# akanazawa/human_dynamics

Hardware: NVIDIA H100
Metric: frames/sec (ResNet->f_movie->SMPL LBS) (higher is better)
Workload: dtype f32 (wgmma 3x fp16 head/remainder split, fp32 two-level accumulate)

## Files before the change

### human_dynamics_b200/csrc/conv_tc.cu

```cuda
#include <cuda.h>
#include <cuda_fp16.h>
#include <cstdlib>
#include "conv_common.cuh"
#include "tc_ptx.cuh"

namespace hd {
namespace {

constexpr int BM = 128;
constexpr int A_TILE_BYTES = BM * 128;
constexpr int BOX_BYTES = 64 * 128;
constexpr int W_PROD = 8;
constexpr int STAGE_OUT = 1, STAGE_PAIR = 2;

using namespace ptx;

template <bool SPLIT, bool HALF, bool ASPLIT, int BN, bool RES = false, bool SHORT = false>
struct Cfg {
  static_assert(BN == 64 || (BN == 128 && HALF && ASPLIT), "128-wide N tiles: pre-split fp16 path only");
  static_assert(!RES || ASPLIT, "residual by TMA: pre-split fp16 path only");
  static_assert(!SHORT || (BN == 64 && HALF && ASPLIT), "two CTAs per SM: 64-wide pre-split fp16 tiles only");
  static constexpr int CTAS = SHORT ? 2 : 1;
  static constexpr int PROD_THREADS = BN == 128 || SHORT ? 128 : 256;
  static constexpr int NUM_THREADS = 256 + PROD_THREADS;
  static constexpr int ROW_STEP = PROD_THREADS / 8;
  static constexpr int ROWS = BM / ROW_STEP;
  static constexpr int PROD_REGS = SHORT ? 32 : BN == 128 ? 40 : 104, CONS_REGS = SHORT ? 104 : BN == 128 ? 232 : 152;
  static_assert(CTAS * (256 * CONS_REGS + PROD_THREADS * PROD_REGS) <= 65536, "setmaxnreg split beyond the register file");
  static constexpr int NACC = BN / 2;
  static constexpr int STAGES = SHORT ? 1 : BN == 128 ? (RES ? 2 : 3) : (RES ? 3 : 4);
  static constexpr int BKE = HALF ? 64 : 32;
  static constexpr int B_TILE_BYTES = BN * 128;
  static constexpr int B_OFFSET = (SPLIT ? 2 : 1) * A_TILE_BYTES;
  static constexpr int STAGE_BYTES = (SPLIT ? 2 : 1) * (A_TILE_BYTES + B_TILE_BYTES);
  static constexpr int RES_OFFSET = STAGES * STAGE_BYTES;
  static constexpr int RES_SLOT_BYTES = RES || SHORT ? 64 * BN * 4 : 0;
  static constexpr int STG_OFFSET = SHORT ? RES_OFFSET : RES_OFFSET + 2 * RES_SLOT_BYTES;
  static constexpr int STG_BYTES = ASPLIT ? 2 * BOX_BYTES : 0;
  static_assert(!SHORT || STG_BYTES == RES_SLOT_BYTES, "SHORT: the staging buffer is the residual slot");
  static constexpr int BAR_OFFSET = SHORT ? RES_OFFSET + 2 * RES_SLOT_BYTES : STG_OFFSET + 2 * STG_BYTES;
  static constexpr int SMEM_BYTES = BAR_OFFSET + 128 + 1024;
  static_assert(SMEM_BYTES <= 232448, "dynamic shared memory beyond the 227 KB a CTA can opt into");
  static_assert(CTAS * (SMEM_BYTES + 1024) <= 233472, "CTAS CTAs (and the 1 KB each reserves) beyond an SM's 228 KB");
  static constexpr int PF = HALF ? 2 : 3;
  static constexpr int V = HALF ? 2 : 1;
};

template <int R>
struct RowState {
  int n[R], iy[R], ix[R];
};

template <bool SPLIT, int PCH, bool HALF, bool GATHER, bool ASPLIT, int BN, bool RES, bool SHORT>
__global__ void __launch_bounds__((Cfg<SPLIT, HALF, ASPLIT, BN, RES, SHORT>::NUM_THREADS), (Cfg<SPLIT, HALF, ASPLIT, BN, RES, SHORT>::CTAS))
conv_gemm_tc_kernel(const ConvParams p, const __grid_constant__ CUtensorMap tmap_hi, const __grid_constant__ CUtensorMap tmap_lo,
                    const __grid_constant__ CUtensorMap tmap_res, const __grid_constant__ CUtensorMap tmap_out,
                    const __grid_constant__ CUtensorMap tmap_out_hi, const __grid_constant__ CUtensorMap tmap_out_lo, const int stage) {
  using C = Cfg<SPLIT, HALF, ASPLIT, BN, RES, SHORT>;
  constexpr bool MEM_STAMPS = BN == 128 || SHORT;
  constexpr int BKE = C::BKE, PF = C::PF, V = C::V, STAGES = C::STAGES, R = C::ROWS, RS = C::ROW_STEP, NA = C::NACC;
  extern __shared__ uint8_t smem_raw[];
  const uint32_t smem_base = (smem_u32(smem_raw) + 1023u) & ~1023u;
  uint8_t *smem = smem_raw + (smem_base - smem_u32(smem_raw));
  const uint32_t bar_base = smem_base + C::BAR_OFFSET;
  auto full_bar = [&](int s) { return bar_base + 8u * s; };
  auto empty_bar = [&](int s) { return bar_base + 8u * (STAGES + s); };
  auto res_bar = [&](int g) { return bar_base + 8u * (2 * STAGES + g); };

  const int warp = threadIdx.x >> 5, lane = threadIdx.x & 31;
  const int num_k = (GATHER ? p.K_pad : p.K) / BKE;
  const int tiles_n = (p.Cout + BN - 1) / BN;
  const int num_tiles = ((p.M + BM - 1) / BM) * tiles_n;
  const int my_tiles = (num_tiles - (int)blockIdx.x + (int)gridDim.x - 1) / (int)gridDim.x;

  if (threadIdx.x == 0) {
    for (int s = 0; s < STAGES; ++s) {
      mbar_init(full_bar(s), ASPLIT ? C::PROD_THREADS + 1 : 9);
      mbar_init(empty_bar(s), 8);
    }
    if (RES) for (int g = 0; g < 2; ++g) mbar_init(res_bar(g), 1);
    asm volatile("fence.mbarrier_init.release.cluster;" ::: "memory");
  }
  __syncthreads();
  const int xmode = p.dbg ? (int)p.dbg[15] : 0;

  if (warp >= W_PROD) {
    asm volatile("setmaxnreg.dec.sync.aligned.u32 %0;" ::"n"(C::PROD_REGS));
    const int t = threadIdx.x - W_PROD * 32;
    const int j = t & 7;
    const int rb = t >> 3;
    const uint32_t sw_off = (uint32_t)((j ^ (rb & 7)) << 4);
    const bool prof = p.dbg != nullptr && blockIdx.x == 0 && t == 0;
    long long t_wait = 0, t_start = prof && !MEM_STAMPS ? clock64() : 0;
    if (MEM_STAMPS && prof) { p.dbg[0] = clock64(); p.dbg[1] = 0; }
    auto wait_empty = [&](int s, uint32_t ph) {
      if (MEM_STAMPS && prof) p.dbg[1] -= clock64();
      const long long tw0 = !MEM_STAMPS && prof ? clock64() : 0;
      mbar_wait(empty_bar(s), ph ^ 1u);
      if (!MEM_STAMPS && prof) t_wait += clock64() - tw0;
      if (MEM_STAMPS && prof) p.dbg[1] += clock64();
    };
    const int total = my_tiles * num_k;
    auto load_b = [&](int s, int ti, int kc) {
      if (t != 0) return;
      const int n0 = (((int)blockIdx.x + ti * (int)gridDim.x) % tiles_n) * BN;
      const uint32_t b_hi = smem_base + s * C::STAGE_BYTES + C::B_OFFSET;
      if (xmode & 2) { mbar_arrive(full_bar(s)); return; }
      const int boxes = (BN == 128 && n0 + 64 < p.Cout) ? 2 : 1;
      mbar_arrive_expect_tx(full_bar(s), (SPLIT ? 2 : 1) * boxes * BOX_BYTES);
      for (int b = 0; b < boxes; ++b) {
        tma_load_2d(b_hi + b * BOX_BYTES, &tmap_hi, full_bar(s), kc * BKE, n0 + 64 * b);
        if (SPLIT) tma_load_2d(b_hi + C::B_TILE_BYTES + b * BOX_BYTES, &tmap_lo, full_bar(s), kc * BKE, n0 + 64 * b);
      }
    };

    auto enter_tile = [&](int ti, RowState<R> &rs) {
      const int tile = (int)blockIdx.x + ti * (int)gridDim.x;
      const int m0 = (tile / tiles_n) * BM;
      const int hw = p.Ho * p.Wo;
#pragma unroll
      for (int i = 0; i < R; ++i) {
        const int m = m0 + rb + RS * i;
        if (m < p.M) {
          const int n = m / hw;
          const int r = m - n * hw;
          const int oy = r / p.Wo, ox = r - oy * p.Wo;
          rs.n[i] = n; rs.iy[i] = oy * p.stride - p.pad_t; rs.ix[i] = ox * p.stride - p.pad_l;
        } else {
          rs.n[i] = -1; rs.iy[i] = 0; rs.ix[i] = 0;
        }
      }
    };
    if constexpr (ASPLIT) {
      const __half *ihi = reinterpret_cast<const __half *>(p.in_hi);
      const __half *ilo = reinterpret_cast<const __half *>(p.in_lo);
      if (SHORT || (!p.planes && p.KH * p.KW <= 32 && (long long)p.n_img * p.H * p.W * p.in_ld < (1ll << 31))) {
        const uint32_t off0 = (uint32_t)rb * 128u + sw_off;
        int base[R];
        uint32_t mask[R];
        int kc = 0, ti = 0, tap = 0, ci0 = 0, kx = 0, ky = 0, tap_off = 0;
        for (int q = 0; q < total; ++q) {
          if (kc == 0) {
            const int tile = (int)blockIdx.x + ti * (int)gridDim.x;
            const int m0 = (tile / tiles_n) * BM + rb;
            const int hw = p.Ho * p.Wo;
#pragma unroll
            for (int i = 0; i < R; ++i) {
              const int m = m0 + RS * i;
              uint32_t mk = 0;
              int b = 0;
              if (m < p.M) {
                const int n = m / hw;
                const int r = m - n * hw;
                const int oy = r / p.Wo, ox = r - oy * p.Wo;
                const int iy0 = oy * p.stride - p.pad_t, ix0 = ox * p.stride - p.pad_l;
                b = ((n * p.H + iy0) * p.W + ix0) * p.in_ld + j * 8;
                int t = 0;
                for (int yy = 0; yy < p.KH; ++yy)
                  for (int xx = 0; xx < p.KW; ++xx, ++t)
                    if ((unsigned)(iy0 + yy) < (unsigned)p.H && (unsigned)(ix0 + xx) < (unsigned)p.W) mk |= 1u << t;
              }
              base[i] = SHORT && !(mk & 1u) ? -1 : b;
              mask[i] = mk;
            }
            tap = 0; ci0 = 0; kx = 0; ky = 0; tap_off = 0;
          }
          const int s = q % STAGES;
          const uint32_t ph = (uint32_t)(q / STAGES) & 1u;
          wait_empty(s, ph);
          load_b(s, ti, kc);
          const uint32_t a_hi = smem_base + s * C::STAGE_BYTES + off0;
          const int eo = SHORT ? ci0 : tap_off + ci0;
#pragma unroll
          for (int i = 0; i < R; ++i) {
            const bool ok = SHORT ? base[i] >= 0 : (mask[i] >> tap) & 1u;
            const int e = ok ? base[i] + eo : 0;
            cp_async16(a_hi + i * RS * 128, ihi + e, ok ? 16u : 0u);
            if (SPLIT) cp_async16(a_hi + A_TILE_BYTES + i * RS * 128, ilo + e, ok ? 16u : 0u);
          }
          asm volatile("cp.async.mbarrier.arrive.noinc.shared::cta.b64 [%0];" ::"r"(full_bar(s)) : "memory");
          ci0 += BKE;
          if (ci0 == p.Cin) {
            ci0 = 0; ++tap;
            if (++kx == p.KW) { kx = 0; ++ky; }
            tap_off = (ky * p.W + kx) * p.in_ld;
          }
          if (++kc == num_k) { kc = 0; ++ti; }
        }
      } else if (!SHORT && p.planes && (long long)p.n_img * p.H * p.W * p.in_ld < (1ll << 31)) {
        const uint32_t off0 = (uint32_t)rb * 128u + sw_off;
        const int jt = j >> 2;
        const int row_step = 2 * p.W * (int)p.in_ld;
        int base[R];
        int kc = 0, ti = 0;
        for (int q = 0; q < total; ++q) {
          if (kc == 0) {
            const int tile = (int)blockIdx.x + ti * (int)gridDim.x;
            const int m0 = (tile / tiles_n) * BM + rb;
            const int hw = p.Ho * p.Wo;
#pragma unroll
            for (int i = 0; i < R; ++i) {
              const int m = m0 + RS * i;
              int b = -1;
              if (m < p.M) {
                const int n = m / hw;
                const int r = m - n * hw;
                const int oy = r / p.Wo, ox = r - oy * p.Wo;
                b = ((n * p.H + oy * p.stride + jt) * p.W + ox * p.stride) * (int)p.in_ld + (j & 3) * 8;
              }
              base[i] = b;
            }
          }
          const int s = q % STAGES;
          const uint32_t ph = (uint32_t)(q / STAGES) & 1u;
          wait_empty(s, ph);
          load_b(s, ti, kc);
          const uint32_t a_hi = smem_base + s * C::STAGE_BYTES + off0;
          const bool tap_ok = 2 * kc + jt < 7;
          const int eo = kc * row_step;
#pragma unroll
          for (int i = 0; i < R; ++i) {
            const bool ok = tap_ok && base[i] >= 0;
            const int e = ok ? base[i] + eo : 0;
            cp_async16_ca(a_hi + i * RS * 128, ihi + e, ok ? 16u : 0u);
            if (SPLIT) cp_async16_ca(a_hi + A_TILE_BYTES + i * RS * 128, ilo + e, ok ? 16u : 0u);
          }
          asm volatile("cp.async.mbarrier.arrive.noinc.shared::cta.b64 [%0];" ::"r"(full_bar(s)) : "memory");
          if (++kc == num_k) { kc = 0; ++ti; }
        }
      } else if (!SHORT) {
      RowState<R> rs;
      int kc = 0, ti = 0;
      for (int q = 0; q < total; ++q) {
        if (kc == 0) enter_tile(ti, rs);
        const int s = q % STAGES;
        const uint32_t ph = (uint32_t)(q / STAGES) & 1u;
        wait_empty(s, ph);
        load_b(s, ti, kc);
        const int kb = kc * BKE;
        const int tap = p.planes ? 2 * kc + (j >> 2) : kb / p.Cin;
        const int ci = p.planes ? (j & 3) * 8 : kb - tap * p.Cin + j * 8;
        const int ky = tap / p.KW, kx = tap - ky * p.KW;
        const bool tap_ok = !p.planes || tap < 7;
        const uint32_t a_hi = smem_base + s * C::STAGE_BYTES, a_lo = a_hi + A_TILE_BYTES;
#pragma unroll
        for (int i = 0; i < R; ++i) {
          const int iy = rs.iy[i] + ky, ix = rs.ix[i] + kx;
          const bool ok = tap_ok && rs.n[i] >= 0 && iy >= 0 && iy < p.H && ix >= 0 && ix < p.W;
          const size_t e = ok ? ((size_t)((size_t)rs.n[i] * p.H + iy) * p.W + ix) * p.in_ld + ci : 0;
          const uint32_t off = (uint32_t)(rb + RS * i) * 128u + sw_off;
          if (p.planes) {
            cp_async16_ca(a_hi + off, ihi + e, ok ? 16u : 0u);
            if (SPLIT) cp_async16_ca(a_lo + off, ilo + e, ok ? 16u : 0u);
          } else {
            cp_async16(a_hi + off, ihi + e, ok ? 16u : 0u);
            if (SPLIT) cp_async16(a_lo + off, ilo + e, ok ? 16u : 0u);
          }
        }
        asm volatile("cp.async.mbarrier.arrive.noinc.shared::cta.b64 [%0];" ::"r"(full_bar(s)) : "memory");
        if (++kc == num_k) { kc = 0; ++ti; }
      }
      }
      cp_async_commit();
      cp_async_wait<0>();
      if (prof) { p.dbg[0] = clock64() - (MEM_STAMPS ? p.dbg[0] : t_start); if (!MEM_STAMPS) p.dbg[1] = t_wait; }
    } else {
    RowState<R> pf_rs, st_rs;
    float4 ring[PF][4 * V];
    uint32_t vmask[PF];
    int pf_kc = 0, pf_ti = 0;
    auto prefetch = [&](float4 *dst, uint32_t &vm) {
      if (pf_kc == 0) enter_tile(pf_ti, pf_rs);
      if (GATHER) {
        const int seg = p.KW * p.Cin, segp = (seg + 7) & ~7;
        const int g8 = (pf_kc * BKE + j * (4 * V)) / 8;
        const int gpr = segp >> 3;
        const int ky = g8 / gpr, r0 = (g8 - ky * gpr) * 8;
        vm = 0;
#pragma unroll
        for (int i = 0; i < 4; ++i) {
          const int iy = pf_rs.iy[i] + ky;
          const bool okr = pf_rs.n[i] >= 0 && ky < p.KH && iy >= 0 && iy < p.H;
          const int c0 = pf_rs.ix[i] * p.Cin + r0;
          const float *src = p.in + ((size_t)((size_t)(okr ? pf_rs.n[i] : 0) * p.H + (okr ? iy : 0)) * p.W) * p.in_ld + c0;
          const int rowlen = p.W * p.Cin;
          float xs[8];
#pragma unroll
          for (int e = 0; e < 8; ++e) {
            const bool ok = okr && (r0 + e) < seg && (c0 + e) >= 0 && (c0 + e) < rowlen;
            xs[e] = ok ? __ldg(src + e) : 0.f;
          }
          dst[i * V] = make_float4(xs[0], xs[1], xs[2], xs[3]);
          dst[i * V + V - 1] = make_float4(xs[4], xs[5], xs[6], xs[7]);
          if (pf_rs.n[i] >= 0) vm |= 1u << i;
        }
        if (++pf_kc == num_k) { pf_kc = 0; ++pf_ti; }
        return;
      }
      const int kb = pf_kc * BKE;
      const int tap = kb / p.Cin, ci = kb - tap * p.Cin + j * (4 * V);
      const int ky = tap / p.KW, kx = tap - ky * p.KW;
      vm = 0;
#pragma unroll
      for (int i = 0; i < 4; ++i) {
        const int iy = pf_rs.iy[i] + ky, ix = pf_rs.ix[i] + kx;
        const bool ok = pf_rs.n[i] >= 0 && iy >= 0 && iy < p.H && ix >= 0 && ix < p.W;
        if (ok && !(xmode & 4)) {
          const float4 *src = reinterpret_cast<const float4 *>(p.in + ((size_t)((size_t)pf_rs.n[i] * p.H + iy) * p.W + ix) * p.in_ld + ci);
#pragma unroll
          for (int v = 0; v < V; ++v) dst[i * V + v] = __ldg(src + v);
          vm |= 1u << i;
        } else {
#pragma unroll
          for (int v = 0; v < V; ++v) dst[i * V + v] = make_float4(0.f, 0.f, 0.f, 0.f);
        }
      }
      if (++pf_kc == num_k) { pf_kc = 0; ++pf_ti; }
    };
    int st_kc = 0, st_ti = 0;
    auto consume = [&](int q, float4 *cur, uint32_t vm) {
      if (st_kc == 0) enter_tile(st_ti, st_rs);
      const int s = q % STAGES;
      const uint32_t ph = (uint32_t)(q / STAGES) & 1u;
      long long tw0 = prof ? clock64() : 0;
      mbar_wait(empty_bar(s), ph ^ 1u);
      if (prof) t_wait += clock64() - tw0;
      load_b(s, st_ti, st_kc);
      uint8_t *a_hi = smem + s * C::STAGE_BYTES;
      uint8_t *a_lo = a_hi + A_TILE_BYTES;
      const int pci = p.pre_scale ? (st_kc * BKE) % p.Cin + j * (4 * V) : 0;
#pragma unroll
      for (int i = 0; i < 4; ++i) {
        float xs[4 * V];
#pragma unroll
        for (int v = 0; v < V; ++v) {
          const float4 x = cur[i * V + v];
          xs[4 * v] = x.x; xs[4 * v + 1] = x.y; xs[4 * v + 2] = x.z; xs[4 * v + 3] = x.w;
        }
        if (p.pre_scale && (vm & (1u << i))) {
          const size_t po = (size_t)(p.pre_img_stride != 0 ? st_rs.n[i] : 0) * p.pre_img_stride + pci;
#pragma unroll
          for (int v = 0; v < V; ++v) {
            const float4 sc = __ldg(reinterpret_cast<const float4 *>(p.pre_scale + po) + v);
            const float4 sh = __ldg(reinterpret_cast<const float4 *>(p.pre_shift + po) + v);
            xs[4 * v] = xs[4 * v] * sc.x + sh.x; xs[4 * v + 1] = xs[4 * v + 1] * sc.y + sh.y;
            xs[4 * v + 2] = xs[4 * v + 2] * sc.z + sh.z; xs[4 * v + 3] = xs[4 * v + 3] * sc.w + sh.w;
          }
          if (p.pre_relu) {
#pragma unroll
            for (int e = 0; e < 4 * V; ++e) xs[e] = fmaxf(xs[e], 0.f);
          }
        }
        uint32_t h[4], l[4];
        if (!HALF) {
#pragma unroll
          for (int e = 0; e < 4; ++e) {
            const float hf = rn_tf32(xs[e]);
            h[e] = __float_as_uint(hf);
            l[e] = __float_as_uint(rn_tf32(xs[e] - hf));
          }
        } else {
#pragma unroll
          for (int e = 0; e < 4; ++e) split_f16x2(xs[2 * e], xs[2 * e + 1], h[e], l[e]);
        }
        const uint32_t off = (uint32_t)(rb + 32 * i) * 128u + sw_off;
        if (xmode & 1) continue;
        *reinterpret_cast<uint4 *>(a_hi + off) = make_uint4(h[0], h[1], h[2], h[3]);
        if (SPLIT) *reinterpret_cast<uint4 *>(a_lo + off) = make_uint4(l[0], l[1], l[2], l[3]);
      }
      asm volatile("fence.proxy.async.shared::cta;" ::: "memory");
      __syncwarp();
      if (lane == 0) mbar_arrive(full_bar(s));
      if (++st_kc == num_k) { st_kc = 0; ++st_ti; }
    };
#pragma unroll
    for (int u = 0; u < PF - 1; ++u)
      if (u < total) prefetch(ring[u], vmask[u]);
    for (int q0 = 0; q0 < total; q0 += PF) {
#pragma unroll
      for (int u = 0; u < PF; ++u) {
        const int q = q0 + u;
        if (q < total) {
          if (q + PF - 1 < total) prefetch(ring[(u + PF - 1) % PF], vmask[(u + PF - 1) % PF]);
          consume(q, ring[u], vmask[u]);
        }
      }
    }
    if (prof) { p.dbg[0] = clock64() - t_start; p.dbg[1] = t_wait; }
    }
  } else if (warp < W_PROD) {
    asm volatile("setmaxnreg.inc.sync.aligned.u32 %0;" ::"n"(C::CONS_REGS));
    const int wg = warp >> 2;
    const bool prof = p.dbg != nullptr && blockIdx.x == 0 && threadIdx.x == 0;
    long long t_wait = 0, t_start = prof && !MEM_STAMPS && !RES ? clock64() : 0;
    if ((RES || MEM_STAMPS) && prof) p.dbg[2] = clock64();
    if (prof) { p.dbg[3] = 0; p.dbg[4] = 0; p.dbg[5] = 0; p.dbg[6] = 0; }
    const int hw = p.Ho * p.Wo;
    const int frow = wg * 64 + (warp & 3) * 16 + (lane >> 2);
    const int fcol = 2 * (lane & 3);
    float acc[NA], accx[SPLIT ? NA : 1], sums_[SHORT ? 1 : NA];
    float *const sums = SHORT ? acc : sums_;
#pragma unroll
    for (int i = 0; i < NA; ++i) {
      acc[i] = 0.f;
      if constexpr (SPLIT) accx[i] = 0.f;
    }
    uint8_t *res_sm = smem + C::RES_OFFSET + wg * C::RES_SLOT_BYTES;
    const bool res_issuer = RES && (threadIdx.x & 127) == 0;
    const bool stg_issuer = ASPLIT && (threadIdx.x & 127) == 0;
    auto load_res = [&](int ti) {
      const int tile = (int)blockIdx.x + ti * (int)gridDim.x;
      const int r0 = (tile / tiles_n) * BM + 64 * wg, c0 = (tile % tiles_n) * BN;
      const int cols = p.Cout - c0 < BN ? p.Cout - c0 : BN;
      const int boxes = r0 < p.M ? (cols + 31) / 32 : 0;
      const uint32_t slot = smem_base + C::RES_OFFSET + wg * C::RES_SLOT_BYTES;
      mbar_arrive_expect_tx(res_bar(wg), boxes * (64 * 128));
      for (int b = 0; b < boxes; ++b) tma_load_2d(slot + b * (64 * 128), &tmap_res, res_bar(wg), c0 + 32 * b, r0);
    };
    if (res_issuer && my_tiles > 0) load_res(0);
    int q = 0;
    for (int ti = 0; ti < my_tiles; ++ti) {
      if (!SHORT) {
#pragma unroll
        for (int i = 0; i < NA; ++i) sums[i] = 0.f;
      }
      for (int kc = 0; kc < num_k; ++kc, ++q) {
        const int s = q % STAGES;
        const uint32_t ph = (uint32_t)(q / STAGES) & 1u;
        const bool group_start = (kc % PCH) == 0;
        if (MEM_STAMPS && prof) p.dbg[3] -= clock64();
        const long long tw0 = !MEM_STAMPS && prof ? clock64() : 0;
        mbar_wait(full_bar(s), ph);
        if (!MEM_STAMPS && prof) t_wait += clock64() - tw0;
        if (MEM_STAMPS && prof) p.dbg[3] += clock64();
        if (ASPLIT) asm volatile("fence.proxy.async.shared::cta;" ::: "memory");
        const uint32_t a_hi = smem_base + s * C::STAGE_BYTES + wg * (64 * 128);
        const uint32_t a_lo = a_hi + A_TILE_BYTES;
        const uint32_t b_hi = smem_base + s * C::STAGE_BYTES + C::B_OFFSET;
        const uint32_t b_lo = b_hi + C::B_TILE_BYTES;
        const uint64_t da_hi = make_smem_desc(a_hi), da_lo = make_smem_desc(a_lo);
        const uint64_t db_hi = make_smem_desc(b_hi), db_lo = make_smem_desc(b_lo);
        fence_regs(acc);
        if constexpr (SPLIT) fence_regs(accx);
        wgmma_fence();
#pragma unroll
        for (int k = 0; k < 4; ++k) {
          const uint64_t adv = (uint64_t)((k * 32) >> 4);
          if constexpr (BN == 128) {
            if constexpr (SPLIT) {
              wgmma_m64n128k16_f16(accx, da_lo + adv, db_hi + adv, (kc | k) != 0);
              wgmma_m64n128k16_f16(accx, da_hi + adv, db_lo + adv, 1u);
            }
            wgmma_m64n128k16_f16(acc, da_hi + adv, db_hi + adv, !(group_start && k == 0));
          } else if constexpr (HALF) {
            if constexpr (SPLIT) {
              wgmma_m64n64k16_f16(accx, da_lo + adv, db_hi + adv, (kc | k) != 0);
              wgmma_m64n64k16_f16(accx, da_hi + adv, db_lo + adv, 1u);
            }
            wgmma_m64n64k16_f16(acc, da_hi + adv, db_hi + adv, !(group_start && k == 0));
          } else {
            if constexpr (SPLIT) {
              wgmma_m64n64k8_tf32(accx, da_lo + adv, db_hi + adv, (kc | k) != 0);
              wgmma_m64n64k8_tf32(accx, da_hi + adv, db_lo + adv, 1u);
            }
            wgmma_m64n64k8_tf32(acc, da_hi + adv, db_hi + adv, !(group_start && k == 0));
          }
        }
        wgmma_commit();
        wgmma_wait<0>();
        fence_regs(acc);
        if constexpr (SPLIT) fence_regs(accx);
        __syncwarp();
        if (lane == 0) mbar_arrive(empty_bar(s));
        if (!SHORT && ((kc % PCH) == PCH - 1 || kc == num_k - 1)) {
#pragma unroll
          for (int i = 0; i < NA; ++i) sums[i] += acc[i];
        }
      }
      if (SHORT) {
#pragma unroll
        for (int i = 0; i < NA; ++i) acc[i] = __fadd_rn(0.f, acc[i]);
      }
      if constexpr (SPLIT) {
#pragma unroll
        for (int i = 0; i < NA; ++i) sums[i] += accx[i] * (HALF ? (1.0f / 2048.0f) : 1.0f);
      }
      if (prof) p.dbg[4] -= clock64();
      const int tile = (int)blockIdx.x + ti * (int)gridDim.x;
      const int m0 = (tile / tiles_n) * BM, n0 = (tile % tiles_n) * BN;
      if (RES && prof) p.dbg[5] -= clock64();
      if (RES) mbar_wait(res_bar(wg), (uint32_t)ti & 1u);
      if (RES && prof) p.dbg[5] += clock64();
      auto row_geom = [&](int m, int &n_img, int &oy, int &ox) {
        n_img = 0; oy = 0; ox = 0;
        if (p.out_sub || (!RES && p.res && !(p.res_stride == 1 && p.res_H == p.Ho && p.res_W == p.Wo))) {
          n_img = m / hw;
          const int r = m - n_img * hw;
          oy = r / p.Wo; ox = r - oy * p.Wo;
        }
      };
      auto res_row = [&](int m, int n_img, int oy, int ox) -> const float * {
        if (RES || !p.res) return nullptr;
        const size_t rr = (p.res_stride == 1 && p.res_H == p.Ho && p.res_W == p.Wo)
                              ? (size_t)m
                              : ((size_t)n_img * p.res_H + (size_t)oy * p.res_stride) * p.res_W + (size_t)ox * p.res_stride;
        return p.res + rr * p.res_ld;
      };
      auto out_row = [&](int m, int n_img, int oy, int ox) -> float * {
        if (!p.out) return nullptr;
        if (!p.out_sub) return p.out + (size_t)m * p.out_ld;
        if (oy % p.out_sub != 0 || ox % p.out_sub != 0) return nullptr;
        const int Hs = (p.Ho + p.out_sub - 1) / p.out_sub, Ws = (p.Wo + p.out_sub - 1) / p.out_sub;
        return p.out + ((size_t)((size_t)n_img * Hs + oy / p.out_sub) * Ws + ox / p.out_sub) * p.out_ld;
      };
      auto value2 = [&](int c, const float2 *rs, const float *rrow, float &y0, float &y1) {
        if (p.post_scale) { const float2 sc = __ldg(reinterpret_cast<const float2 *>(p.post_scale + c)); y0 *= sc.x; y1 *= sc.y; }
        if (p.post_shift) { const float2 sh = __ldg(reinterpret_cast<const float2 *>(p.post_shift + c)); y0 += sh.x; y1 += sh.y; }
        if (RES) { const float2 r = *rs; y0 += r.x; y1 += r.y; }
        else if (rrow) { const float2 r = *reinterpret_cast<const float2 *>(rrow + c); y0 += r.x; y1 += r.y; }
        if (p.post_relu) { y0 = fmaxf(y0, 0.f); y1 = fmaxf(y1, 0.f); }
      };
      auto pair2 = [&](int c, float a0, float a1, uint32_t &hh, uint32_t &ll) {
        if (p.post2_scale) { const float2 sc = __ldg(reinterpret_cast<const float2 *>(p.post2_scale + c)); a0 *= sc.x; a1 *= sc.y; }
        if (p.post2_shift) { const float2 sh = __ldg(reinterpret_cast<const float2 *>(p.post2_shift + c)); a0 += sh.x; a1 += sh.y; }
        if (p.post2_relu) { a0 = fmaxf(a0, 0.f); a1 = fmaxf(a1, 0.f); }
        split_f16x2(a0, a1, hh, ll);
      };
      if constexpr (ASPLIT) {
        const bool st32 = (stage & STAGE_OUT) != 0, st2 = (stage & STAGE_PAIR) != 0;
        uint8_t *stg = smem + C::STG_OFFSET + wg * C::STG_BYTES;
        const uint32_t stg_a = smem_base + C::STG_OFFSET + wg * C::STG_BYTES;
        const int r0 = m0 + 64 * wg;
        const uint32_t rsw = (uint32_t)(lane >> 2);
        auto acquire = [&](bool after_out) {
          if (prof) p.dbg[6] -= clock64();
          if (stg_issuer) {
            if (after_out) bulk_wait_read<1>();
            else bulk_wait_read<0>();
          }
          named_bar_sync(3 + wg, 128);
          if (prof) p.dbg[6] += clock64();
        };
#pragma unroll
        for (int cc = 0; cc < BN / 64; ++cc) {
          const int c0 = n0 + 64 * cc;
          const bool issue = stg_issuer && r0 < p.M && c0 < p.Cout;
          if (st32 && !RES) acquire(false);
          const bool rok[2] = {m0 + frow < p.M, m0 + frow + 8 < p.M};
          if (st32 && (RES || !p.res)) {
            uint8_t *brow = (RES ? res_sm + 2 * cc * BOX_BYTES : stg) + (frow - 64 * wg) * 128 + 8 * (lane & 1);
            const float *vsc = p.post_scale ? p.post_scale + c0 + fcol : nullptr, *vsh = p.post_shift ? p.post_shift + c0 + fcol : nullptr;
#pragma unroll
            for (int jj = 0; jj < 8; ++jj) {
              const int j = 8 * cc + jj;
              if (c0 + 8 * jj + fcol >= p.Cout) continue;
              const uint32_t piece = (uint32_t)(2 * (jj & 3) + ((lane & 3) >> 1)) ^ rsw;
              const float2 sc = vsc ? __ldg(reinterpret_cast<const float2 *>(vsc + 8 * jj)) : make_float2(0.f, 0.f);
              const float2 sh = vsh ? __ldg(reinterpret_cast<const float2 *>(vsh + 8 * jj)) : make_float2(0.f, 0.f);
#pragma unroll
              for (int h = 0; h < 2; ++h) {
                if (!rok[h]) continue;
                float2 *f32 = reinterpret_cast<float2 *>(brow + h * 1024 + (jj >> 2) * BOX_BYTES + piece * 16);
                float y0 = sums[4 * j + 2 * h], y1 = sums[4 * j + 2 * h + 1];
                if (vsc) { y0 = __fmul_rn(y0, sc.x); y1 = __fmul_rn(y1, sc.y); }
                if (vsh) { y0 = __fadd_rn(y0, sh.x); y1 = __fadd_rn(y1, sh.y); }
                if (RES) { const float2 r = *f32; y0 = __fadd_rn(y0, r.x); y1 = __fadd_rn(y1, r.y); }
                if (p.post_relu) { y0 = fmaxf(y0, 0.f); y1 = fmaxf(y1, 0.f); }
                *f32 = make_float2(y0, y1);
                sums[4 * j + 2 * h] = y0; sums[4 * j + 2 * h + 1] = y1;
              }
            }
          } else {
#pragma unroll
          for (int h = 0; h < 2; ++h) {
            const int m = m0 + frow + 8 * h;
            if (m >= p.M) continue;
            int n_img, oy, ox;
            row_geom(m, n_img, oy, ox);
            const float *rrow = res_row(m, n_img, oy, ox);
            float *orow = st32 ? nullptr : out_row(m, n_img, oy, ox);
            uint8_t *brow = (RES ? res_sm + 2 * cc * BOX_BYTES : stg) + (frow - 64 * wg + 8 * h) * 128 + 8 * (lane & 1);
#pragma unroll
            for (int jj = 0; jj < 8; ++jj) {
              const int j = 8 * cc + jj;
              const int c = n0 + 8 * j + fcol;
              if (c >= p.Cout) continue;
              const uint32_t piece = (uint32_t)(2 * (jj & 3) + ((lane & 3) >> 1)) ^ rsw;
              float2 *f32 = reinterpret_cast<float2 *>(brow + (jj >> 2) * BOX_BYTES + piece * 16);
              float y0 = sums[4 * j + 2 * h], y1 = sums[4 * j + 2 * h + 1];
              value2(c, f32, rrow, y0, y1);
              if (st32) *f32 = make_float2(y0, y1);
              else if (orow) *reinterpret_cast<float2 *>(orow + c) = make_float2(y0, y1);
              sums[4 * j + 2 * h] = y0; sums[4 * j + 2 * h + 1] = y1;
            }
          }
          }
          if (st32) {
            fence_proxy_async();
            named_bar_sync(3 + wg, 128);
            if (issue) {
              const uint32_t src = RES ? smem_base + C::RES_OFFSET + wg * C::RES_SLOT_BYTES + 2 * cc * BOX_BYTES : stg_a;
              tma_store_2d(&tmap_out, src, c0, r0);
              if (c0 + 32 < p.Cout) tma_store_2d(&tmap_out, src + BOX_BYTES, c0 + 32, r0);
            }
            if (stg_issuer) bulk_commit();
          }
          if (p.out_hi) {
            if (st2) acquire(RES && st32 && !SHORT);
            if (st2) {
              uint8_t *brow = stg + (frow - 64 * wg) * 128 + 4 * (lane & 3);
              const float *vsc = p.post2_scale ? p.post2_scale + c0 + fcol : nullptr, *vsh = p.post2_shift ? p.post2_shift + c0 + fcol : nullptr;
#pragma unroll
              for (int jj = 0; jj < 8; ++jj) {
                const int j = 8 * cc + jj;
                if (c0 + 8 * jj + fcol >= p.Cout) continue;
                const float2 sc = vsc ? __ldg(reinterpret_cast<const float2 *>(vsc + 8 * jj)) : make_float2(0.f, 0.f);
                const float2 sh = vsh ? __ldg(reinterpret_cast<const float2 *>(vsh + 8 * jj)) : make_float2(0.f, 0.f);
#pragma unroll
                for (int h = 0; h < 2; ++h) {
                  if (!rok[h]) continue;
                  float a0 = sums[4 * j + 2 * h], a1 = sums[4 * j + 2 * h + 1];
                  if (vsc) { a0 = __fmul_rn(a0, sc.x); a1 = __fmul_rn(a1, sc.y); }
                  if (vsh) { a0 = __fadd_rn(a0, sh.x); a1 = __fadd_rn(a1, sh.y); }
                  if (p.post2_relu) { a0 = fmaxf(a0, 0.f); a1 = fmaxf(a1, 0.f); }
                  uint32_t hh, ll;
                  split_f16x2(a0, a1, hh, ll);
                  uint32_t *hs = reinterpret_cast<uint32_t *>(brow + h * 1024 + (((uint32_t)jj ^ rsw) * 16));
                  hs[0] = hh;
                  if (SPLIT) hs[BOX_BYTES / 4] = ll;
                }
              }
            } else {
#pragma unroll
            for (int h = 0; h < 2; ++h) {
              const int m = m0 + frow + 8 * h;
              if (m >= p.M) continue;
              __half *hrow = reinterpret_cast<__half *>(p.out_hi) + (size_t)m * p.out2_ld;
              __half *lrow = SPLIT ? reinterpret_cast<__half *>(p.out_lo) + (size_t)m * p.out2_ld : nullptr;
              uint8_t *brow = stg + (frow - 64 * wg + 8 * h) * 128 + 4 * (lane & 3);
#pragma unroll
              for (int jj = 0; jj < 8; ++jj) {
                const int j = 8 * cc + jj;
                const int c = n0 + 8 * j + fcol;
                if (c >= p.Cout) continue;
                uint32_t hh, ll;
                pair2(c, sums[4 * j + 2 * h], sums[4 * j + 2 * h + 1], hh, ll);
                if (st2) {
                  uint32_t *hs = reinterpret_cast<uint32_t *>(brow + (((uint32_t)jj ^ rsw) * 16));
                  hs[0] = hh;
                  if (SPLIT) hs[BOX_BYTES / 4] = ll;
                } else {
                  *reinterpret_cast<uint32_t *>(hrow + c) = hh;
                  if (SPLIT) *reinterpret_cast<uint32_t *>(lrow + c) = ll;
                }
              }
            }
            }
            if (st2) {
              fence_proxy_async();
              named_bar_sync(3 + wg, 128);
              if (issue) {
                tma_store_2d(&tmap_out_hi, stg_a, c0, r0);
                if (SPLIT) tma_store_2d(&tmap_out_lo, stg_a + BOX_BYTES, c0, r0);
              }
              if (stg_issuer) bulk_commit();
            }
          }
        }
      } else {
#pragma unroll
      for (int h = 0; h < 2; ++h) {
        const int m = m0 + frow + 8 * h;
        if (m >= p.M) continue;
        int n_img, oy, ox;
        row_geom(m, n_img, oy, ox);
        const float *rrow = res_row(m, n_img, oy, ox);
        float *orow = out_row(m, n_img, oy, ox);
        __half *hrow = p.out_hi ? reinterpret_cast<__half *>(p.out_hi) + (size_t)m * p.out2_ld : nullptr;
        __half *lrow = SPLIT && p.out_hi ? reinterpret_cast<__half *>(p.out_lo) + (size_t)m * p.out2_ld : nullptr;
#pragma unroll
        for (int j = 0; j < BN / 8; ++j) {
          const int c = n0 + 8 * j + fcol;
          if (c >= p.Cout) continue;
          const bool two = c + 1 < p.Cout;
          float y[2] = {sums[4 * j + 2 * h], sums[4 * j + 2 * h + 1]};
          if (p.vec_out) {
            value2(c, nullptr, rrow, y[0], y[1]);
            if (orow) *reinterpret_cast<float2 *>(orow + c) = make_float2(y[0], y[1]);
            if (hrow) {
              uint32_t hh, ll;
              pair2(c, y[0], y[1], hh, ll);
              *reinterpret_cast<uint32_t *>(hrow + c) = hh;
              if (SPLIT) *reinterpret_cast<uint32_t *>(lrow + c) = ll;
            }
          } else {
#pragma unroll
            for (int e = 0; e < 2; ++e) {
              if (e == 1 && !two) break;
              float v = y[e];
              if (p.post_scale) v *= __ldg(p.post_scale + c + e);
              if (p.post_shift) v += __ldg(p.post_shift + c + e);
              if (rrow) v += rrow[c + e];
              if (p.post_relu) v = fmaxf(v, 0.f);
              if (orow) orow[c + e] = v;
            }
          }
        }
      }
      }
      if (RES && ti + 1 < my_tiles) {
        if (prof) p.dbg[6] -= clock64();
        named_bar_sync(1 + wg, 128);
        if (res_issuer) {
          if (SHORT) {
            if (stage) bulk_wait_read<0>();
          } else if (stage & STAGE_OUT) {
            if (stage & STAGE_PAIR) bulk_wait_read<1>();
            else bulk_wait_read<0>();
          }
          load_res(ti + 1);
        }
        if (prof) p.dbg[6] += clock64();
      }
      if (prof) p.dbg[4] += clock64();
    }
    if (stg_issuer) bulk_wait_all();
    if (prof) { p.dbg[2] = clock64() - (RES || MEM_STAMPS ? p.dbg[2] : t_start); if (!MEM_STAMPS) p.dbg[3] = t_wait; }
  }
}

typedef CUresult (*EncodeTiledFn)(CUtensorMap *, CUtensorMapDataType, cuuint32_t, void *, const cuuint64_t *, const cuuint64_t *,
                                  const cuuint32_t *, const cuuint32_t *, CUtensorMapInterleave, CUtensorMapSwizzle,
                                  CUtensorMapL2promotion, CUtensorMapFloatOOBfill);

EncodeTiledFn get_encode_fn() {
  static EncodeTiledFn fn = nullptr;
  static bool tried = false;
  if (!tried) {
    tried = true;
    void *ptr = nullptr;
    cudaDriverEntryPointQueryResult qres;
    cudaError_t e = cudaGetDriverEntryPoint("cuTensorMapEncodeTiled", &ptr, cudaEnableDefault, &qres);
    if (e == cudaSuccess && qres == cudaDriverEntryPointSuccess) fn = reinterpret_cast<EncodeTiledFn>(ptr);
    else (void)cudaGetLastError();
  }
  return fn;
}

constexpr int kMaxDevices = 64;

int encode_epilogue_map(CUtensorMap *tm, bool fp16, const void *base, int cols, int rows, long long ld_bytes, const char *what) {
  EncodeTiledFn fn = get_encode_fn();
  if (!fn) { set_last_error_text("cuTensorMapEncodeTiled unavailable (no CUDA driver?)"); return HD_ERR_UNSUPPORTED; }
  const cuuint64_t gdim[2] = {(cuuint64_t)cols, (cuuint64_t)rows};
  const cuuint64_t gstride[1] = {(cuuint64_t)ld_bytes};
  const cuuint32_t box[2] = {fp16 ? 64u : 32u, 64u};
  const cuuint32_t estr[2] = {1u, 1u};
  CUresult r = fn(tm, fp16 ? CU_TENSOR_MAP_DATA_TYPE_FLOAT16 : CU_TENSOR_MAP_DATA_TYPE_FLOAT32, 2, const_cast<void *>(base), gdim, gstride,
                  box, estr, CU_TENSOR_MAP_INTERLEAVE_NONE, CU_TENSOR_MAP_SWIZZLE_128B, CU_TENSOR_MAP_L2_PROMOTION_L2_128B,
                  CU_TENSOR_MAP_FLOAT_OOB_FILL_NONE);
  if (r != CUDA_SUCCESS) {
    char msg[96];
    snprintf(msg, sizeof(msg), "cuTensorMapEncodeTiled (%s) failed with CUresult %d", what, (int)r);
    set_last_error_text(msg);
    return HD_ERR_CUDA;
  }
  return HD_OK;
}

template <bool SPLIT, int PCH, bool HALF, bool GATHER = false, bool ASPLIT = false, int BN = 64, bool RES = false, bool SHORT = false>
int launch_tc(const ConvParams &p, const hd_conv_desc *d, cudaStream_t st) {
  using C = Cfg<SPLIT, HALF, ASPLIT, BN, RES, SHORT>;
  static bool configured[kMaxDevices] = {};
  static int num_sms[kMaxDevices] = {};
  int dev = 0;
  cudaGetDevice(&dev);
  if (dev < 0 || dev >= kMaxDevices) { set_last_error_text("conv_gemm_tc: device ordinal out of range"); return HD_ERR_UNSUPPORTED; }
  if (!configured[dev]) {
    cudaError_t e = cudaFuncSetAttribute(conv_gemm_tc_kernel<SPLIT, PCH, HALF, GATHER, ASPLIT, BN, RES, SHORT>,
                                         cudaFuncAttributeMaxDynamicSharedMemorySize, C::SMEM_BYTES);
    if (e != cudaSuccess) { set_last_error("conv_gemm_tc attr", e); return HD_ERR_CUDA; }
    cudaDeviceGetAttribute(&num_sms[dev], cudaDevAttrMultiProcessorCount, dev);
    if (num_sms[dev] <= 0) { set_last_error_text("conv_gemm_tc: no multiprocessor count"); return HD_ERR_CUDA; }
    configured[dev] = true;
  }
  alignas(64) CUtensorMap thi, tlo;
  const void *mhi = d->tmap_hi_n64 ? d->tmap_hi_n64 : d->tmap_hi;
  const void *mlo = d->tmap_hi_n64 ? d->tmap_lo_n64 : d->tmap_lo;
  memcpy(&thi, mhi, sizeof(CUtensorMap));
  memcpy(&tlo, mlo ? mlo : mhi, sizeof(CUtensorMap));
  alignas(64) CUtensorMap tres, tout, tohi, tolo;
  memcpy(&tres, &thi, sizeof(CUtensorMap));
  memcpy(&tout, &thi, sizeof(CUtensorMap));
  memcpy(&tohi, &thi, sizeof(CUtensorMap));
  memcpy(&tolo, &thi, sizeof(CUtensorMap));
  int rc = HD_OK;
  if (RES) rc = encode_epilogue_map(&tres, false, p.res, p.Cout, p.M, p.res_ld * 4, "residual");
  int stage = 0;
  if (ASPLIT && p.out && !p.out_sub) {
    stage |= STAGE_OUT;
    if (rc == HD_OK) rc = encode_epilogue_map(&tout, false, p.out, p.Cout, p.M, p.out_ld * 4, "output");
  }
  if (ASPLIT && p.out_hi && p.out2_ld % 8 == 0) {
    stage |= STAGE_PAIR;
    if (rc == HD_OK) rc = encode_epilogue_map(&tohi, true, p.out_hi, p.Cout, p.M, p.out2_ld * 2, "output head");
    if (rc == HD_OK && SPLIT) rc = encode_epilogue_map(&tolo, true, p.out_lo, p.Cout, p.M, p.out2_ld * 2, "output remainder");
  }
  if (rc != HD_OK) return rc;
  const int num_tiles = ceil_div(p.M, BM) * ceil_div(p.Cout, BN);
  const int ctas = C::CTAS * num_sms[dev];
  dim3 grid(num_tiles < ctas ? num_tiles : ctas);
  conv_gemm_tc_kernel<SPLIT, PCH, HALF, GATHER, ASPLIT, BN, RES, SHORT>
      <<<grid, C::NUM_THREADS, C::SMEM_BYTES, st>>>(p, thi, tlo, tres, tout, tohi, tolo, stage);
  return check_launch("conv_gemm_tc_kernel");
}

bool wide_n_tile(const ConvParams &p) {
  if (p.Cout <= 64) return false;
  int dev = 0, sms = 0;
  cudaGetDevice(&dev);
  cudaDeviceGetAttribute(&sms, cudaDevAttrMultiProcessorCount, dev);
  if (sms <= 0) return true;
  const long long m_tiles = ceil_div(p.M, BM);
  const long long w128 = (m_tiles * ceil_div(p.Cout, 128) + sms - 1) / sms, w64 = (m_tiles * ceil_div(p.Cout, 64) + sms - 1) / sms;
  return 16 * w128 <= 9 * w64;
}

template <bool SPLIT, bool RES>
bool short_k_two_ctas() {
  using C = Cfg<SPLIT, true, true, 64, RES, true>;
  static int two[kMaxDevices] = {};
  int dev = 0;
  cudaGetDevice(&dev);
  if (dev < 0 || dev >= kMaxDevices) return false;
  if (two[dev] == 0) {
    const auto kernel = conv_gemm_tc_kernel<SPLIT, 2, true, false, true, 64, RES, true>;
    int n = 0;
    if (cudaFuncSetAttribute(kernel, cudaFuncAttributeMaxDynamicSharedMemorySize, C::SMEM_BYTES) != cudaSuccess ||
        cudaOccupancyMaxActiveBlocksPerMultiprocessor(&n, kernel, C::NUM_THREADS, C::SMEM_BYTES) != cudaSuccess) {
      (void)cudaGetLastError();
      n = 0;
    }
    two[dev] = n >= 2 ? 1 : -1;
  }
  return two[dev] > 0;
}

template <bool SPLIT>
int launch_conv_f16(const ConvParams &p, const hd_conv_desc *d, cudaStream_t st) {
  if (p.in_hi && p.planes) {
    if (p.Cin != 32 || p.KH != 8 || p.KW != 1 || p.stride != 2 || p.pad_t != 0 || p.pad_l != 0 || p.in_ld != 4 || p.Cout > 64 ||
        p.W % 2 != 0 || 2 * (p.Wo - 1) + 8 > p.W || 2 * (p.Ho - 1) + 7 > p.H || !aligned16(p.in_hi) || !aligned16(p.in_lo) || p.pre_scale) {
      set_last_error_text("hd_conv_gemm(tc planes): needs the conv1 plane geometry (Cin 32, KH 8, KW 1, stride 2, in_ld 4, even W)");
      return HD_ERR_INVALID;
    }
    return launch_tc<SPLIT, 2, true, false, true>(p, d, st);
  }
  if (p.in_hi) {
    if (p.Cin % 64 != 0 || p.K % 64 != 0 || p.in_ld % 8 != 0 || !aligned16(p.in_hi) || !aligned16(p.in_lo) || p.pre_scale) {
      set_last_error_text("hd_conv_gemm(tc split-A): needs Cin % 64 == 0, in_ld % 8 == 0, aligned in_hi/in_lo, no prologue");
      return HD_ERR_INVALID;
    }
    const bool res_rows = p.res && p.res_stride == 1 && p.res_H == p.Ho && p.res_W == p.Wo && p.K <= 8 * 64;
    const bool short_k = p.K <= 2 * 64 && p.KH * p.KW == 1 && (long long)p.n_img * p.H * p.W * p.in_ld < (1ll << 31) &&
                         (p.res ? res_rows : p.out_hi != nullptr);
    if (short_k && (res_rows ? short_k_two_ctas<SPLIT, true>() : short_k_two_ctas<SPLIT, false>()))
      return res_rows ? launch_tc<SPLIT, 2, true, false, true, 64, true, true>(p, d, st)
                      : launch_tc<SPLIT, 2, true, false, true, 64, false, true>(p, d, st);
    if (wide_n_tile(p))
      return res_rows ? launch_tc<SPLIT, 2, true, false, true, 128, true>(p, d, st) : launch_tc<SPLIT, 2, true, false, true, 128>(p, d, st);
    return res_rows ? launch_tc<SPLIT, 2, true, false, true, 64, true>(p, d, st) : launch_tc<SPLIT, 2, true, false, true>(p, d, st);
  }
  if (p.Cin % 64 != 0) {
    const int segp = (p.KW * p.Cin + 7) & ~7;
    if (p.K_pad % 64 != 0 || p.K_pad < p.KH * segp || p.Cout > 64 || p.pre_scale || p.in_ld != p.Cin) {
      set_last_error_text("hd_conv_gemm(tc gather): needs K_pad % 64 == 0, K_pad >= KH*roundup8(KW*Cin), Cout <= 64, dense pixels, no prologue");
      return HD_ERR_INVALID;
    }
    return launch_tc<SPLIT, 2, true, true>(p, d, st);
  }
  if (!p.in || p.in_ld % 4 != 0 || !aligned16(p.in) || p.K % 64 != 0 ||
      (p.pre_scale && (!aligned16(p.pre_scale) || !aligned16(p.pre_shift) || p.pre_img_stride % 4 != 0))) {
    set_last_error_text("hd_conv_gemm(tc): needs Cin % 32 (tf32) / % 64 (fp16) == 0 and 16-byte aligned input / prologue vectors");
    return HD_ERR_INVALID;
  }
  return launch_tc<SPLIT, 2, true>(p, d, st);
}

}

int launch_conv_tc(const ConvParams &p, const hd_conv_desc *d, cudaStream_t st) {
  const bool heads = d->impl == HD_IMPL_TC_1XF16;
  const bool split_b = d->impl != HD_IMPL_TC_1XTF32 && !heads;
  if (!d->tmap_hi || (split_b && !d->tmap_lo) || (!d->tmap_hi_n64 && d->tmap_lo_n64) || (d->tmap_hi_n64 && split_b && !d->tmap_lo_n64)) {
    set_last_error_text("hd_conv_gemm(tc): missing tensor maps (tmap_hi/tmap_lo, and tmap_hi_n64/tmap_lo_n64 together or not at all)");
    return HD_ERR_INVALID;
  }
  const bool half = d->impl == HD_IMPL_TC_3XF16 || heads;
  if (p.out_sub) {
    const bool res_plain = !p.res || (p.res_stride == 1 && p.res_H == p.Ho && p.res_W == p.Wo);
    const bool maps = (!p.res || d->tmap_res) && (!p.out_hi || (d->tmap_out_hi && (heads || d->tmap_out_lo)));
    if (!p.in_hi || p.planes || !maps || !res_plain || p.Cout % 32 != 0 || (d->flags & HD_CONV_NO_TMA_EPILOGUE)) {
      set_last_error_text("hd_conv_gemm: out_subsample needs the activation-map epilogue (pre-split input, Cout % 32 == 0, activation maps given)");
      return HD_ERR_UNSUPPORTED;
    }
  }
  if ((p.out_hi || p.in_hi) && (!half || !p.vec_out)) {
    set_last_error_text("hd_conv_gemm(tc): pre-split activations need impl 3 / 4 and 16-byte aligned, 4-column-multiple outputs");
    return HD_ERR_INVALID;
  }
  if (half) return heads ? launch_conv_f16<false>(p, d, st) : launch_conv_f16<true>(p, d, st);
  if (!p.in || p.Cin % 32 != 0 || p.in_ld % 4 != 0 || !aligned16(p.in) || p.K % 32 != 0 ||
      (p.pre_scale && (!aligned16(p.pre_scale) || !aligned16(p.pre_shift) || p.pre_img_stride % 4 != 0))) {
    set_last_error_text("hd_conv_gemm(tc): needs Cin % 32 (tf32) / % 64 (fp16) == 0 and 16-byte aligned input / prologue vectors");
    return HD_ERR_INVALID;
  }
  return d->impl != HD_IMPL_TC_1XTF32 ? launch_tc<true, 2, false>(p, d, st) : launch_tc<false, 8, false>(p, d, st);
}

}

extern "C" int hd_make_weight_tmap(const void *w_nk, int rows, int k_pad, int box_rows, int elem_bytes, void *tmap_out) {
  HD_REQUIRE(w_nk && tmap_out && rows > 0 && k_pad > 0 && (elem_bytes == 4 || elem_bytes == 2) && k_pad % (128 / elem_bytes) == 0 &&
                 box_rows == 64 && rows % box_rows == 0 && hd::aligned16(w_nk),
             "hd_make_weight_tmap: bad arguments");
  hd::EncodeTiledFn fn = hd::get_encode_fn();
  if (!fn) { hd::set_last_error_text("cuTensorMapEncodeTiled unavailable (no CUDA driver?)"); return HD_ERR_UNSUPPORTED; }
  alignas(64) CUtensorMap tm;
  const cuuint64_t gdim[2] = {(cuuint64_t)k_pad, (cuuint64_t)rows};
  const cuuint64_t gstride[1] = {(cuuint64_t)k_pad * (cuuint64_t)elem_bytes};
  const cuuint32_t box[2] = {(cuuint32_t)(128 / elem_bytes), (cuuint32_t)box_rows};
  const cuuint32_t estr[2] = {1u, 1u};
  CUresult r = fn(&tm, elem_bytes == 4 ? CU_TENSOR_MAP_DATA_TYPE_FLOAT32 : CU_TENSOR_MAP_DATA_TYPE_FLOAT16, 2, const_cast<void *>(w_nk),
                  gdim, gstride, box, estr, CU_TENSOR_MAP_INTERLEAVE_NONE, CU_TENSOR_MAP_SWIZZLE_128B,
                  CU_TENSOR_MAP_L2_PROMOTION_L2_128B, CU_TENSOR_MAP_FLOAT_OOB_FILL_NONE);
  if (r != CUDA_SUCCESS) {
    char msg[96];
    snprintf(msg, sizeof(msg), "cuTensorMapEncodeTiled failed with CUresult %d", (int)r);
    hd::set_last_error_text(msg);
    return HD_ERR_CUDA;
  }
  memcpy(tmap_out, &tm, sizeof(tm));
  return HD_OK;
}

extern "C" int hd_make_act_tmap(const void *base, long long rows, int cols, long long ld_elems, int elem_bytes, void *tmap_out) {
  HD_REQUIRE(base && tmap_out && rows > 0 && cols > 0 && ld_elems >= cols && (elem_bytes == 4 || elem_bytes == 2) && hd::aligned16(base) &&
                 (ld_elems * elem_bytes) % 16 == 0,
             "hd_make_act_tmap: bad arguments (16-byte aligned base and row pitch required)");
  hd::EncodeTiledFn fn = hd::get_encode_fn();
  if (!fn) { hd::set_last_error_text("cuTensorMapEncodeTiled unavailable (no CUDA driver?)"); return HD_ERR_UNSUPPORTED; }
  alignas(64) CUtensorMap tm;
  const cuuint64_t gdim[2] = {(cuuint64_t)cols, (cuuint64_t)rows};
  const cuuint64_t gstride[1] = {(cuuint64_t)ld_elems * (cuuint64_t)elem_bytes};
  const cuuint32_t box[2] = {32u, 128u};
  const cuuint32_t estr[2] = {1u, 1u};
  CUresult r = fn(&tm, elem_bytes == 4 ? CU_TENSOR_MAP_DATA_TYPE_FLOAT32 : CU_TENSOR_MAP_DATA_TYPE_FLOAT16, 2, const_cast<void *>(base), gdim,
                  gstride, box, estr, CU_TENSOR_MAP_INTERLEAVE_NONE, elem_bytes == 4 ? CU_TENSOR_MAP_SWIZZLE_128B : CU_TENSOR_MAP_SWIZZLE_64B,
                  CU_TENSOR_MAP_L2_PROMOTION_L2_128B, CU_TENSOR_MAP_FLOAT_OOB_FILL_NONE);
  if (r != CUDA_SUCCESS) {
    char msg[96];
    snprintf(msg, sizeof(msg), "cuTensorMapEncodeTiled (activation) failed with CUresult %d", (int)r);
    hd::set_last_error_text(msg);
    return HD_ERR_CUDA;
  }
  memcpy(tmap_out, &tm, sizeof(tm));
  return HD_OK;
}
```

Before: 13310.

## Route mid-K 1x1 residual convs to two-CTA kernel with smem-parked partial sums

Adds a MIDK variant of the two-CTA-per-SM short-K kernel for 1x1 convolutions with K of 192 or 256 and a residual. Instead of holding separate running-sum registers, each PCH chunk's accumulator is added into a float2 slot in the shared-memory staging/residual buffer. The residual TMA load is deferred until the last chunk has been read back. The aim is to let these mid-K layers run at two CTAs per SM with low register counts, at the cost of extra shared-memory round trips and named-barrier syncs per chunk.

```diff
diff --git a/human_dynamics_b200/csrc/conv_tc.cu b/human_dynamics_b200/csrc/conv_tc.cu
--- a/human_dynamics_b200/csrc/conv_tc.cu
+++ b/human_dynamics_b200/csrc/conv_tc.cu
@@ -51,12 +51,13 @@
   int n[R], iy[R], ix[R];
 };
 
-template <bool SPLIT, int PCH, bool HALF, bool GATHER, bool ASPLIT, int BN, bool RES, bool SHORT>
+template <bool SPLIT, int PCH, bool HALF, bool GATHER, bool ASPLIT, int BN, bool RES, bool SHORT, bool MIDK>
 __global__ void __launch_bounds__((Cfg<SPLIT, HALF, ASPLIT, BN, RES, SHORT>::NUM_THREADS), (Cfg<SPLIT, HALF, ASPLIT, BN, RES, SHORT>::CTAS))
 conv_gemm_tc_kernel(const ConvParams p, const __grid_constant__ CUtensorMap tmap_hi, const __grid_constant__ CUtensorMap tmap_lo,
                     const __grid_constant__ CUtensorMap tmap_res, const __grid_constant__ CUtensorMap tmap_out,
                     const __grid_constant__ CUtensorMap tmap_out_hi, const __grid_constant__ CUtensorMap tmap_out_lo, const int stage) {
   using C = Cfg<SPLIT, HALF, ASPLIT, BN, RES, SHORT>;
+  static_assert(!MIDK || SHORT, "running sums in the slot: the two-CTA configuration only");
   constexpr bool MEM_STAMPS = BN == 128 || SHORT;
   constexpr int BKE = C::BKE, PF = C::PF, V = C::V, STAGES = C::STAGES, R = C::ROWS, RS = C::ROW_STEP, NA = C::NACC;
   extern __shared__ uint8_t smem_raw[];
@@ -417,7 +418,7 @@
       mbar_arrive_expect_tx(res_bar(wg), boxes * (64 * 128));
       for (int b = 0; b < boxes; ++b) tma_load_2d(slot + b * (64 * 128), &tmap_res, res_bar(wg), c0 + 32 * b, r0);
     };
-    if (res_issuer && my_tiles > 0) load_res(0);
+    if (!MIDK && res_issuer && my_tiles > 0) load_res(0);
     int q = 0;
     for (int ti = 0; ti < my_tiles; ++ti) {
       if (!SHORT) {
@@ -476,8 +477,47 @@
 #pragma unroll
           for (int i = 0; i < NA; ++i) sums[i] += acc[i];
         }
-      }
-      if (SHORT) {
+        if (MIDK && ((kc % PCH) == PCH - 1 || kc == num_k - 1)) {
+          if (prof) p.dbg[4] -= clock64();
+          const bool first = kc < PCH, last = kc == num_k - 1;
+          if (first) {
+            if (prof) p.dbg[6] -= clock64();
+            if (stg_issuer) bulk_wait_read<0>();
+            named_bar_sync(3 + wg, 128);
+            if (prof) p.dbg[6] += clock64();
+          }
+          uint8_t *brow = res_sm + (frow - 64 * wg) * 128 + 8 * (lane & 1);
+          auto parked = [&](int i) {
+            const int jj = i >> 2, h = (i >> 1) & 1;
+            const uint32_t piece = (uint32_t)(2 * (jj & 3) + ((lane & 3) >> 1)) ^ (uint32_t)(lane >> 2);
+            return reinterpret_cast<float2 *>(brow + h * 1024 + (jj >> 2) * BOX_BYTES + piece * 16);
+          };
+          if (first) {
+#pragma unroll
+            for (int i = 0; i < NA; i += 2) *parked(i) = make_float2(__fadd_rn(0.f, acc[i]), __fadd_rn(0.f, acc[i + 1]));
+          } else if (!last) {
+#pragma unroll
+            for (int i = 0; i < NA; i += 2) {
+              float2 *f = parked(i);
+              const float2 s = *f;
+              *f = make_float2(__fadd_rn(s.x, acc[i]), __fadd_rn(s.y, acc[i + 1]));
+            }
+          } else {
+#pragma unroll
+            for (int i = 0; i < NA; i += 2) {
+              const float2 s = *parked(i);
+              acc[i] = __fadd_rn(s.x, acc[i]); acc[i + 1] = __fadd_rn(s.y, acc[i + 1]);
+            }
+          }
+          if (RES && last) {
+            fence_proxy_async();
+            named_bar_sync(1 + wg, 128);
+            if (res_issuer) load_res(ti);
+          }
+          if (prof) p.dbg[4] += clock64();
+        }
+      }
+      if (SHORT && !MIDK) {
 #pragma unroll
         for (int i = 0; i < NA; ++i) acc[i] = __fadd_rn(0.f, acc[i]);
       }
@@ -708,7 +748,7 @@
         }
       }
       }
-      if (RES && ti + 1 < my_tiles) {
+      if (RES && !MIDK && ti + 1 < my_tiles) {
         if (prof) p.dbg[6] -= clock64();
         named_bar_sync(1 + wg, 128);
         if (res_issuer) {
@@ -768,7 +808,8 @@
   return HD_OK;
 }
 
-template <bool SPLIT, int PCH, bool HALF, bool GATHER = false, bool ASPLIT = false, int BN = 64, bool RES = false, bool SHORT = false>
+template <bool SPLIT, int PCH, bool HALF, bool GATHER = false, bool ASPLIT = false, int BN = 64, bool RES = false, bool SHORT = false,
+          bool MIDK = false>
 int launch_tc(const ConvParams &p, const hd_conv_desc *d, cudaStream_t st) {
   using C = Cfg<SPLIT, HALF, ASPLIT, BN, RES, SHORT>;
   static bool configured[kMaxDevices] = {};
@@ -777,7 +818,7 @@
   cudaGetDevice(&dev);
   if (dev < 0 || dev >= kMaxDevices) { set_last_error_text("conv_gemm_tc: device ordinal out of range"); return HD_ERR_UNSUPPORTED; }
   if (!configured[dev]) {
-    cudaError_t e = cudaFuncSetAttribute(conv_gemm_tc_kernel<SPLIT, PCH, HALF, GATHER, ASPLIT, BN, RES, SHORT>,
+    cudaError_t e = cudaFuncSetAttribute(conv_gemm_tc_kernel<SPLIT, PCH, HALF, GATHER, ASPLIT, BN, RES, SHORT, MIDK>,
                                          cudaFuncAttributeMaxDynamicSharedMemorySize, C::SMEM_BYTES);
     if (e != cudaSuccess) { set_last_error("conv_gemm_tc attr", e); return HD_ERR_CUDA; }
     cudaDeviceGetAttribute(&num_sms[dev], cudaDevAttrMultiProcessorCount, dev);
@@ -810,7 +851,7 @@
   const int num_tiles = ceil_div(p.M, BM) * ceil_div(p.Cout, BN);
   const int ctas = C::CTAS * num_sms[dev];
   dim3 grid(num_tiles < ctas ? num_tiles : ctas);
-  conv_gemm_tc_kernel<SPLIT, PCH, HALF, GATHER, ASPLIT, BN, RES, SHORT>
+  conv_gemm_tc_kernel<SPLIT, PCH, HALF, GATHER, ASPLIT, BN, RES, SHORT, MIDK>
       <<<grid, C::NUM_THREADS, C::SMEM_BYTES, st>>>(p, thi, tlo, tres, tout, tohi, tolo, stage);
   return check_launch("conv_gemm_tc_kernel");
 }
@@ -826,7 +867,7 @@
   return 16 * w128 <= 9 * w64;
 }
 
-template <bool SPLIT, bool RES>
+template <bool SPLIT, bool RES, bool MIDK>
 bool short_k_two_ctas() {
   using C = Cfg<SPLIT, true, true, 64, RES, true>;
   static int two[kMaxDevices] = {};
@@ -834,7 +875,7 @@
   cudaGetDevice(&dev);
   if (dev < 0 || dev >= kMaxDevices) return false;
   if (two[dev] == 0) {
-    const auto kernel = conv_gemm_tc_kernel<SPLIT, 2, true, false, true, 64, RES, true>;
+    const auto kernel = conv_gemm_tc_kernel<SPLIT, 2, true, false, true, 64, RES, true, MIDK>;
     int n = 0;
     if (cudaFuncSetAttribute(kernel, cudaFuncAttributeMaxDynamicSharedMemorySize, C::SMEM_BYTES) != cudaSuccess ||
         cudaOccupancyMaxActiveBlocksPerMultiprocessor(&n, kernel, C::NUM_THREADS, C::SMEM_BYTES) != cudaSuccess) {
@@ -862,11 +903,13 @@
       return HD_ERR_INVALID;
     }
     const bool res_rows = p.res && p.res_stride == 1 && p.res_H == p.Ho && p.res_W == p.Wo && p.K <= 8 * 64;
-    const bool short_k = p.K <= 2 * 64 && p.KH * p.KW == 1 && (long long)p.n_img * p.H * p.W * p.in_ld < (1ll << 31) &&
-                         (p.res ? res_rows : p.out_hi != nullptr);
-    if (short_k && (res_rows ? short_k_two_ctas<SPLIT, true>() : short_k_two_ctas<SPLIT, false>()))
+    const bool lean_1x1 = p.KH * p.KW == 1 && (long long)p.n_img * p.H * p.W * p.in_ld < (1ll << 31);
+    const bool short_k = p.K <= 2 * 64 && lean_1x1 && (p.res ? res_rows : p.out_hi != nullptr);
+    if (short_k && (res_rows ? short_k_two_ctas<SPLIT, true, false>() : short_k_two_ctas<SPLIT, false, false>()))
       return res_rows ? launch_tc<SPLIT, 2, true, false, true, 64, true, true>(p, d, st)
                       : launch_tc<SPLIT, 2, true, false, true, 64, false, true>(p, d, st);
+    const bool mid_k = p.K > 2 * 64 && p.K <= 4 * 64 && lean_1x1 && res_rows;
+    if (mid_k && short_k_two_ctas<SPLIT, true, true>()) return launch_tc<SPLIT, 2, true, false, true, 64, true, true, true>(p, d, st);
     if (wide_n_tile(p))
       return res_rows ? launch_tc<SPLIT, 2, true, false, true, 128, true>(p, d, st) : launch_tc<SPLIT, 2, true, false, true, 128>(p, d, st);
     return res_rows ? launch_tc<SPLIT, 2, true, false, true, 64, true>(p, d, st) : launch_tc<SPLIT, 2, true, false, true>(p, d, st);
```

Result: no change. 13340, median of 6 (+0.2%).
